# glmanhtu/vit-ed

Measured on NVIDIA B200. Metric: pair scores/sec (all-pairs ViT-ED), higher is better.
Workload: dtype fp16

## Files before the change

### vit-ed_b200/csrc/attention_tc.cu

```cuda
#include "kernels.h"

namespace vited {

namespace {

constexpr float kLog2e = 1.4426950408889634f;

__device__ __forceinline__ float ex2_ftz(float x) {
  float y;
  asm("ex2.approx.ftz.f32 %0, %1;" : "=f"(y) : "f"(x));
  return y;
}

struct P64 {
  static constexpr int HD = 32;
  static constexpr int RB = 64;
  static constexpr int TROWS = 80;
  static constexpr int TB = TROWS * RB;
  static constexpr int STAGE = 3 * TB;
  static constexpr int NS = 12;
  static constexpr int NT = 4;
  static constexpr int TCOLS = 128;
  static constexpr int OCOL = 96;
  static constexpr int THREADS = 32 * 4 * NT;
  static constexpr int BAR_BYTES = (2 * NS + 4 * NT) * 8 + 16;
  static constexpr int BYTES = 1024 + NS * STAGE + BAR_BYTES;
};

#ifdef VITED_ATTN_TRACE
__device__ unsigned long long g_p64_trace[4 * 64 * 8];
#define TRP(ev) do { if (blockIdx.x == 0 && quarter == 0 && lane == 0 && tk < 64) g_p64_trace[(group * 64 + tk) * 8 + (ev)] = clock64(); } while (0)
#else
#define TRP(ev) do { } while (0)
#endif

struct P64Maps {
  CUtensorMap q_tile, q_row, k_tile, k_row, v_tile, v_row;
};

__global__ void __launch_bounds__(P64::THREADS, 1)
attn_p64_kernel(AttnArgs a, const __grid_constant__ P64Maps maps, int n_units, int mode) {
  using C = P64;
  const int cls_only = mode & 1;
  const bool kv_once = (mode & 2) != 0;
  extern __shared__ uint8_t attn_tc_smem_raw[];
  uint8_t* smem = reinterpret_cast<uint8_t*>((reinterpret_cast<uintptr_t>(attn_tc_smem_raw) + 1023) & ~uintptr_t(1023));
  uint64_t* bars = reinterpret_cast<uint64_t*>(smem + C::NS * C::STAGE);
  uint64_t* full = bars;
  uint64_t* empty = bars + C::NS;
  uint64_t* s_full = bars + 2 * C::NS;
  uint64_t* o_full = s_full + C::NT;
  uint64_t* p_ready = o_full + C::NT;
  uint32_t* tmem_holder = reinterpret_cast<uint32_t*>(p_ready + C::NT);

  const int tid = threadIdx.x, lane = tid & 31;
  const int warp = __shfl_sync(0xffffffffu, tid >> 5, 0);
  const int quarter = warp & 3, group = warp >> 2;
  const int H = a.n_heads;
  const int n_my = (n_units - (int)blockIdx.x + (int)gridDim.x - 1) / (int)gridDim.x;
  const int NK = a.k_has_cls ? 80 : 64;

// ... 110 lines not shown
  } else {
    const float sl2 = a.scale * kLog2e;
    const int row = quarter * 32 + lane;
    const bool warp_active = quarter < 2 ? !cls_only : a.q_has_cls != 0;
    const uint32_t t_col = tmem_base + group * C::TCOLS;
    const uint32_t t_stage = t_col + (static_cast<uint32_t>(quarter * 32) << 16);
    uint32_t ph = 0;
    int tk = 0; (void)tk;
    for (int i = group; i < n_my; i += C::NT, ++tk) {
      const int u = (int)blockIdx.x + i * (int)gridDim.x;
      const int b = u / H, h = u - b * H;
      TRP(0);
      mbar_wait(&s_full[group], ph, 54);
      TRP(1);
      tc_fence_after();
      float l = 1.f;
      if (warp_active) {
        uint32_t v0[32], v1[32];
        uint32_t vc[8];
        tmem_ld_32x32b_x32(t_stage, v0);
        tmem_ld_32x32b_x32(t_stage + 32, v1);
        if (a.k_has_cls) tmem_ld_32x32b_x8(t_stage + 64, vc);
        tmem_ld_wait();
        float mx[4];
#pragma unroll
        for (int j = 0; j < 4; ++j) mx[j] = fmaxf(__uint_as_float(v0[j]), __uint_as_float(v1[j]));
#pragma unroll
        for (int j = 4; j < 32; ++j) mx[j & 3] = fmaxf(mx[j & 3], fmaxf(__uint_as_float(v0[j]), __uint_as_float(v1[j])));
        float mxa = fmaxf(fmaxf(mx[0], mx[1]), fmaxf(mx[2], mx[3]));
        if (a.k_has_cls) mxa = fmaxf(mxa, __uint_as_float(vc[0]));
        const float mneg = -mxa * sl2;
        float sum[4] = {0.f, 0.f, 0.f, 0.f};
        uint32_t pk[32];
#if VITED_SOFTMAX_PACKED
        {
          uint64_t sum2[2] = {0ull, 0ull};
          softmax_exp_pairs<16>(v0, sl2, mneg, pk, sum2);
          softmax_exp_pairs<16>(v1, sl2, mneg, pk + 16, sum2);
          f2_unpack(sum2[0], sum[0], sum[1]);
          f2_unpack(sum2[1], sum[2], sum[3]);
        }
#else
#pragma unroll
        for (int j = 0; j < 16; ++j) {
          const float p0 = ex2_ftz(fmaf(__uint_as_float(v0[2 * j]), sl2, mneg));
          const float p1 = ex2_ftz(fmaf(__uint_as_float(v0[2 * j + 1]), sl2, mneg));
          sum[(2 * j) & 3] += p0; sum[(2 * j + 1) & 3] += p1;
          pk[j] = pack_act(p0, p1);
        }
#pragma unroll
        for (int j = 0; j < 16; ++j) {
          const float p0 = ex2_ftz(fmaf(__uint_as_float(v1[2 * j]), sl2, mneg));
          const float p1 = ex2_ftz(fmaf(__uint_as_float(v1[2 * j + 1]), sl2, mneg));
          sum[(2 * j) & 3] += p0; sum[(2 * j + 1) & 3] += p1;
          pk[16 + j] = pack_act(p0, p1);
        }
#endif
        tmem_st_32x32b_x32(t_stage, pk);
        if (a.k_has_cls) {
          const float pc = ex2_ftz(fmaf(__uint_as_float(vc[0]), sl2, mneg));
          sum[0] += pc;
          uint32_t pc8[8] = {pack_act(pc, 0.f), 0u, 0u, 0u, 0u, 0u, 0u, 0u};
          tmem_st_32x32b_x8(t_stage + 32, pc8);
        }
        l = (sum[0] + sum[1]) + (sum[2] + sum[3]);
        tmem_st_wait();
      }
      tc_fence_before();
      __syncwarp();
      if (lane == 0) mbar_arrive(&p_ready[group]);
      TRP(2);
      mbar_wait(&o_full[group], ph, 55);
      TRP(3);
      tc_fence_after();
      if (warp_active) {
        uint32_t ov[32];
        tmem_ld_32x32b_x32(t_stage + C::OCOL, ov);
        tmem_ld_wait();
        const float inv = 1.f / l;
        size_t orow;
        bool valid = true;
        if (row < 64) { orow = (size_t)b * 64 + row; valid = !cls_only; }
        else if (row == 64 && a.q_has_cls) orow = (size_t)a.n_seq * 64 + b;
        else { valid = false; orow = 0; }
        if (valid) {
          uint4* dst = reinterpret_cast<uint4*>(a.o + orow * a.o_ld + h * C::HD);
#pragma unroll
          for (int c = 0; c < 4; ++c) {
            uint4 w;
            w.x = pack_act(__uint_as_float(ov[8 * c + 0]) * inv, __uint_as_float(ov[8 * c + 1]) * inv);
            w.y = pack_act(__uint_as_float(ov[8 * c + 2]) * inv, __uint_as_float(ov[8 * c + 3]) * inv);
            w.z = pack_act(__uint_as_float(ov[8 * c + 4]) * inv, __uint_as_float(ov[8 * c + 5]) * inv);
            w.w = pack_act(__uint_as_float(ov[8 * c + 6]) * inv, __uint_as_float(ov[8 * c + 7]) * inv);
            dst[c] = w;
          }
        }
      }
      TRP(4);
      ph ^= 1;
    }
  }

  tc_fence_before();
  __syncthreads();
  if (warp == 11) {
    tc_fence_after();
    tmem_dealloc(tmem_base, 512);
  }
}


struct L64 {
  static constexpr int HD = 64;
  static constexpr int RB = 128;
  static constexpr int QB = 128 * RB;
  static constexpr int KVB = 128 * RB;
  static constexpr int STAGE = 2 * KVB;
  static constexpr int NS = 4;
  static constexpr int THREADS = 352;
  static constexpr int GCOLS = 256;
  static constexpr int OCOL = 128;
  static constexpr int BAR_BYTES = 512;
  static constexpr int BYTES = 1024 + 4 * QB + NS * STAGE + BAR_BYTES;
};

#ifdef VITED_ATTN_TRACE
__device__ unsigned long long g_attn_trace[4 * 128 * 4];
#define TR(who, idx, k) do { if (blockIdx.x == 0 && lane == 0 && (idx) < 128) g_attn_trace[((who) * 128 + (idx)) * 4 + (k)] = clock64(); } while (0)
#else
#define TR(who, idx, k) do { } while (0)
#endif
// ... 337 lines not shown
  VITED_CHECK(items < ((size_t)1 << 31), "attention_tc: too many work items");
  static PerDeviceOnce once;
  const int sms = device_sm_count();
  if (once.first())
    VITED_CUDA_OK(cudaFuncSetAttribute(attn_l64_kernel, cudaFuncAttributeMaxDynamicSharedMemorySize, L64::BYTES));
  const uint64_t cols = (uint64_t)a.n_heads * 64;
  const uint64_t q_rows = (uint64_t)a.n_seq * a.nq_patch + (a.q_has_cls ? a.n_seq : 0);
  const uint64_t k_rows = (uint64_t)a.n_kv_seq * a.nk_patch + (a.k_has_cls ? a.n_kv_seq : 0);
  L64Maps maps;
  if (make_tmap_act_2d(&maps.q_tile, a.q, cols, q_rows, (uint64_t)a.q_ld * 2, 64, 128, 128)) return 1;
  if (make_tmap_act_2d(&maps.q_row, a.q, cols, q_rows, (uint64_t)a.q_ld * 2, 64, 1, 128)) return 1;
  if (make_tmap_act_2d(&maps.k_tile, a.k, cols, k_rows, (uint64_t)a.k_ld * 2, 64, 128, 128)) return 1;
  if (make_tmap_act_2d(&maps.k_row, a.k, cols, k_rows, (uint64_t)a.k_ld * 2, 64, 1, 128)) return 1;
  if (make_tmap_act_2d(&maps.v_tile, a.v, cols, k_rows, (uint64_t)a.v_ld * 2, 64, 128, 128)) return 1;
  if (make_tmap_act_2d(&maps.v_row, a.v, cols, k_rows, (uint64_t)a.v_ld * 2, 64, 1, 128)) return 1;
  const unsigned grid = (unsigned)(items < (size_t)sms ? items : (size_t)sms);
  VITED_CUDA_OK(launch_pdl(attn_l64_kernel, dim3(grid), dim3(L64::THREADS), L64::BYTES, stream, a, maps, (int)items));
  VITED_CUDA_OK(cudaGetLastError());
  return 0;
}

static int attention_tc_p64(const AttnArgs& a, int cls_only, cudaStream_t stream);

int attention_tc(const AttnArgs& a, cudaStream_t stream) {
  VITED_CHECK(attention_tc_supported(a), "attention_tc: unsupported shape");
  if (l64_shape(a)) return attention_tc_l64(a, stream);
#ifdef VITED_EXPERIMENTAL
  const char* pr = getenv("VITED_P64_PAIR");
  if (pr != nullptr && atoi(pr) != 0 && attention_pair_supported(a)) return attention_pair(a, stream);
#endif
  return attention_tc_p64(a, 0, stream);
}

bool attention_tc_cls_supported(const AttnArgs& a) { return a.n_heads >= 1 && p64_shape(a) && a.q_has_cls; }
int attention_tc_cls(const AttnArgs& a, cudaStream_t stream) {
  VITED_CHECK(attention_tc_cls_supported(a), "attention_tc_cls: unsupported shape");
  return attention_tc_p64(a, 1, stream);
}

static int attention_tc_p64(const AttnArgs& a, int cls_only, cudaStream_t stream) {
  const size_t units = (size_t)a.n_seq * a.n_heads;
  VITED_CHECK(units < ((size_t)1 << 31), "attention_tc: too many work units");
  static PerDeviceOnce once;
  const int sms = device_sm_count();
  if (once.first())
    VITED_CUDA_OK(cudaFuncSetAttribute(attn_p64_kernel, cudaFuncAttributeMaxDynamicSharedMemorySize, P64::BYTES));
  const uint64_t cols = (uint64_t)a.n_heads * 32;
  const uint64_t q_rows = (uint64_t)a.n_seq * 64 + (a.q_has_cls ? a.n_seq : 0);
  const uint64_t k_rows = (uint64_t)a.n_kv_seq * 64 + (a.k_has_cls ? a.n_kv_seq : 0);
  P64Maps maps;
  if (make_tmap_act_2d(&maps.q_tile, a.q, cols, q_rows, (uint64_t)a.q_ld * 2, 32, 64, 64)) return 1;
  if (make_tmap_act_2d(&maps.q_row, a.q, cols, q_rows, (uint64_t)a.q_ld * 2, 32, 1, 64)) return 1;
  if (make_tmap_act_2d(&maps.k_tile, a.k, cols, k_rows, (uint64_t)a.k_ld * 2, 32, 64, 64)) return 1;
// ... 23 lines not shown
```

### vit-ed_b200/csrc/engine.cu

```cuda
#include "../../include/vited_b200.h"
#include "kernels.h"

#include <cstdarg>
#include <cstdlib>
#include <cstring>
#include <map>
#include <string>
#include <vector>

namespace vited {

static thread_local char g_err[1024] = "";
void set_error(const char* fmt, ...) {
  va_list ap;
  va_start(ap, fmt);
  vsnprintf(g_err, sizeof(g_err), fmt, ap);
  va_end(ap);
}
const char* get_error() { return g_err; }

struct DevBuf {
  void* p = nullptr;
  size_t cap = 0;
  int ensure(size_t bytes) {
// ... 46 lines not shown
  std::vector<DecBlock> dec;
  LNorm norm;
  float* head_w = nullptr;
  float* head_b = nullptr;
  std::vector<void*> owned;
  std::map<std::string, Slot> slots;
  std::vector<std::string> names;
  int loaded = 0;
  int gemm_impl = IMPL_FAST, attn_impl = IMPL_FAST;
  int64_t chunk_rows = 524288;
  int cache_layer0 = 1;
  int prune_tail = 1;
  int fuse_ln = 1;
  int fuse_mlp = 1;
  int kv_budget_mb = 8000;
  int64_t launches = 0;
  int profile = 0;
  std::vector<cudaEvent_t> ev_pool;
  size_t ev_used = 0;
  struct ProfRec { cudaEvent_t ev; int cls; double flops; double bytes; };
  std::vector<ProfRec> recs;
  std::vector<std::string> cls_names;
  std::string profile_json;
  DevBuf x, h, qkv, o, q, delta, hid, col, tok, xsrc, enc_tok, kv, ci, xj, tmp_tok;

  int64_t workspace_bytes() const {
    return (int64_t)(x.cap + h.cap + qkv.cap + o.cap + q.cap + delta.cap + hid.cap + col.cap + tok.cap + xsrc.cap +
                     enc_tok.cap + kv.cap + ci.cap + xj.cap + tmp_tok.cap);
  }
};

namespace vited {

#define TRY(expr)            \
  do {                       \
    if ((expr) != 0) return 1; \
  } while (0)

static int alloc_f32(vited_engine* e, float** p, size_t n) {
  VITED_CUDA_OK(cudaMalloc(p, n * sizeof(float)));
  VITED_CUDA_OK(cudaMemset(*p, 0, n * sizeof(float)));
  e->owned.push_back(*p);
  return 0;
}
static int alloc_act(vited_engine* e, act_t** p, size_t n) {
  VITED_CUDA_OK(cudaMalloc(p, n * sizeof(act_t)));
  VITED_CUDA_OK(cudaMemset(*p, 0, n * sizeof(act_t)));
  e->owned.push_back(*p);
  return 0;
}
static void reg(vited_engine* e, const std::string& name, void* dst, bool to_act, int64_t numel) {
// ... 149 lines not shown
  a.x = x; a.delta = delta; a.gather_src = gsrc; a.gather_idx = gidx; a.gather_off = g_off; a.n_src_seq = n_src;
  a.ln_w = ln ? ln->w : nullptr; a.ln_b = ln ? ln->b : nullptr; a.h = h;
  a.n_seq = n_seq; a.n_patch = e->Ne; a.has_cls = has_cls; a.D = e->D; a.write_x = write_x; a.eps = 1e-6f;
  {
    const double rows = (double)n_seq * (e->Ne + (has_cls ? 1 : 0));
    const double per_row = e->D * (4.0 + (delta ? 2.0 : 0.0) + (write_x ? 4.0 : 0.0) + (ln ? 2.0 : 0.0));
    prof_mark(e, "resid_ln", 0.0, rows * per_row, s);
  }
  return resid_ln(a, s);
}
static int L_attn_self(vited_engine* e, const act_t* qkv, act_t* o, int n_seq, int has_cls, cudaStream_t s) {
  AttnArgs a;
  const int D = e->D;
  a.q = qkv; a.q_ld = 3 * D; a.k = qkv + D; a.k_ld = 3 * D; a.v = qkv + 2 * D; a.v_ld = 3 * D; a.o = o; a.o_ld = D;
  a.n_seq = n_seq; a.n_heads = e->H; a.head_dim = e->hd;
  a.nq_patch = e->Ne; a.q_has_cls = has_cls; a.nk_patch = e->Ne; a.k_has_cls = has_cls;
  a.n_kv_seq = n_seq; a.kv_index = nullptr; a.scale = e->scale;
  {
    const double n = e->Ne + (has_cls ? 1 : 0);
    prof_mark(e, "attn_self", 4.0 * n_seq * n * n * e->D, (double)n_seq * n * e->D * 2.0 * 4.0, s);
  }
  return attention(a, e->attn_impl, s);
}
static int L_attn_cross(vited_engine* e, const act_t* q, const act_t* kv, act_t* o, int n_seq, int n_kv_seq,
                        const int* kv_index, cudaStream_t s) {
  AttnArgs a;
  const int D = e->D;
  a.q = q; a.q_ld = D; a.k = kv; a.k_ld = 2 * D; a.v = kv + D; a.v_ld = 2 * D; a.o = o; a.o_ld = D;
  a.n_seq = n_seq; a.n_heads = e->H; a.head_dim = e->hd;
  a.nq_patch = e->Ne; a.q_has_cls = 1; a.nk_patch = e->Ne; a.k_has_cls = 0;
  a.n_kv_seq = n_kv_seq; a.kv_index = kv_index; a.scale = e->scale;
  prof_mark(e, "attn_cross", 4.0 * n_seq * (double)e->Nd * e->Ne * e->D, (double)n_seq * e->Nd * e->D * 2.0 * 2.0, s);
  return attention(a, e->attn_impl, s);
}

static int L_attn_cls(vited_engine* e, const act_t* q, int q_ld, const act_t* k, const act_t* v, int kv_ld, act_t* o,
                      int n_seq, int k_has_cls, int n_kv_seq, const int* kv_index, cudaStream_t s) {
  AttnArgs a;
  a.q = q; a.q_ld = q_ld; a.k = k; a.k_ld = kv_ld; a.v = v; a.v_ld = kv_ld; a.o = o; a.o_ld = e->D;
  a.n_seq = n_seq; a.n_heads = e->H; a.head_dim = e->hd;
  a.nq_patch = e->Ne; a.q_has_cls = 1; a.nk_patch = e->Ne; a.k_has_cls = k_has_cls;
  a.n_kv_seq = n_kv_seq; a.kv_index = kv_index; a.scale = e->scale;
  prof_mark(e, "attn_cls", 4.0 * n_seq * (double)(e->Ne + k_has_cls) * e->D,
            (double)n_seq * (e->Ne + k_has_cls) * e->D * 2.0 * 2.0, s);
  return attention_cls(a, s);
}
static int L_resid_ln_rows(vited_engine* e, float* x, const act_t* delta, const float* gsrc_cls_rows, const int* gidx,
                           const LNorm* ln, act_t* h, int rows, cudaStream_t s, int g_off = 0) {
  ResidLnArgs a;
  a.x = x; a.delta = delta; a.gather_src = gsrc_cls_rows; a.gather_idx = gidx; a.gather_off = g_off; a.n_src_seq = 0;
  a.ln_w = ln ? ln->w : nullptr; a.ln_b = ln ? ln->b : nullptr; a.h = h;
  a.n_seq = rows; a.n_patch = 1; a.has_cls = 0; a.D = e->D; a.write_x = 1; a.eps = 1e-6f;
  prof_mark(e, "resid_ln", 0.0, (double)rows * e->D * 12.0, s);
  return resid_ln(a, s);
// ... 115 lines not shown
                   s));
    TRY(L_gemm(e, e->h.as<act_t>(), b.kv, e->kv.as<act_t>() + l * per_layer, (int)rows, ACT_NONE, s));
  }
  return 0;
}

static int decode_chunk(vited_engine* e, int P, const int* ci, const int* xj, const float* xsrc, int n_src, int x_off,
                        int n_kv_seq, HeadArgs head, cudaStream_t s) {
  const size_t rows = (size_t)P * e->Nd;
  TRY(ensure_rows(e, rows));
  const size_t D = e->D;
  const size_t cls_off = (size_t)P * e->Ne;
  float* x = e->x.as<float>();
  act_t* h = e->h.as<act_t>();
  act_t* delta = e->delta.as<act_t>();
  act_t* qkv = e->qkv.as<act_t>();
  act_t* o = e->o.as<act_t>();
  act_t* q = e->q.as<act_t>();
  act_t* hid = e->hid.as<act_t>();
  const size_t kv_per_layer = (size_t)n_kv_seq * e->Ne * 2 * D;
  const size_t L = e->dec.size();
  const bool fuse = use_fused_ln(e, rows, e->dec[0].proj);
  bool h_is_norm1 = false;
  for (size_t l = 0; l < L; ++l) {
    DecBlock& b = e->dec[l];
    const bool first = (l == 0);
    const bool tail = e->prune_tail && (l + 1 == L);
    const act_t* kvl = e->kv.as<act_t>() + l * kv_per_layer;
    if (!tail) {
      if (first && e->cache_layer0) {
        TRY(L_resid_ln(e, x, nullptr, xsrc, xj, n_src, &b.norm_cross, h, P, 1, 1, s, x_off));
      } else {
        if (first) TRY(L_resid_ln(e, x, nullptr, xsrc, xj, n_src, &b.norm1, h, P, 1, 1, s, x_off));
        else if (!h_is_norm1) TRY(L_resid_ln(e, x, delta, nullptr, nullptr, 0, &b.norm1, h, P, 1, 1, s));
        TRY(L_gemm(e, h, b.qkv, qkv, (int)rows, ACT_NONE, s));
        TRY(L_attn_self(e, qkv, o, P, 1, s));
        if (fuse) {
          TRY(L_gemm_ln(e, o, b.proj, x, b.norm_cross, h, (int)rows, s));
        } else {
          TRY(L_gemm(e, o, b.proj, delta, (int)rows, ACT_NONE, s));
          TRY(L_resid_ln(e, x, delta, nullptr, nullptr, 0, &b.norm_cross, h, P, 1, 1, s));
        }
      }
      TRY(L_gemm(e, h, b.q, q, (int)rows, ACT_NONE, s));
      TRY(L_attn_cross(e, q, kvl, o, P, n_kv_seq, ci, s));
      h_is_norm1 = false;
      if (fuse && l + 1 < L && use_fused_mlp(e, rows, b.cproj, b.fc1, b.fc2)) {
        TRY(L_cproj_mlp_ln(e, o, b.cproj, b.norm2, b.fc1, b.fc2, x, e->dec[l + 1].norm1, h, (int)rows, s));
        h_is_norm1 = true;
      } else {
        if (fuse) {
          TRY(L_gemm_ln(e, o, b.cproj, x, b.norm2, h, (int)rows, s));
        } else {
          TRY(L_gemm(e, o, b.cproj, delta, (int)rows, ACT_NONE, s));
          TRY(L_resid_ln(e, x, delta, nullptr, nullptr, 0, &b.norm2, h, P, 1, 1, s));
        }
        if (fuse && l + 1 < L) {
          TRY(L_gemm(e, h, b.fc1, hid, (int)rows, ACT_GELU, s));
          TRY(L_gemm_ln(e, hid, b.fc2, x, e->dec[l + 1].norm1, h, (int)rows, s));
          h_is_norm1 = true;
        } else {
          TRY(L_gemm(e, h, b.fc1, hid, (int)rows, ACT_GELU, s));
          TRY(L_gemm(e, hid, b.fc2, delta, (int)rows, ACT_NONE, s));
        }
      }
    } else {
      float* x_c = x + cls_off * D;
      act_t* h_c = h + cls_off * D;
// ... 66 lines not shown
  VITED_CHECK(prop.major == 10, "vited_create: device %d is sm_%d%d; this library contains sm_100a code only", device,
              prop.major, prop.minor);
  vited_engine* e = new vited_engine();
  e->cfg = *cfg;
  e->device = device;
  const char* cr = getenv("VITED_CHUNK_ROWS");
  if (cr && atoll(cr) > 0) e->chunk_rows = atoll(cr);
  const char* fm = getenv("VITED_FUSE_MLP");
  if (fm) e->fuse_mlp = atoi(fm) ? 1 : 0;
  if (build(e) != 0) {
    vited_destroy(e);
    return 1;
  }
  *out = e;
  return 0;
}

void vited_destroy(vited_engine* e) {
  if (!e) return;
  DeviceScope scope(e->device);
  cudaDeviceSynchronize();
  for (void* p : e->owned) cudaFree(p);
  DevBuf* bufs[] = {&e->x, &e->h, &e->qkv, &e->o, &e->q, &e->delta, &e->hid, &e->col, &e->tok, &e->xsrc, &e->enc_tok,
                    &e->kv, &e->ci, &e->xj, &e->tmp_tok};
  for (DevBuf* b : bufs) b->release();
  for (cudaEvent_t ev : e->ev_pool) cudaEventDestroy(ev);
  delete e;
}

int vited_set_option(vited_engine* e, int option, int64_t value) {
  VITED_CHECK(e != nullptr, "null engine");
  switch (option) {
    case VITED_OPT_GEMM_IMPL: e->gemm_impl = value ? IMPL_REF : IMPL_FAST; return 0;
    case VITED_OPT_ATTN_IMPL: e->attn_impl = value == 1 ? IMPL_REF : value == 2 ? IMPL_MMA_SYNC : IMPL_FAST; return 0;
    case VITED_OPT_CHUNK_ROWS:
      VITED_CHECK(value >= 1, "chunk_rows must be positive");
      e->chunk_rows = value;
      return 0;
    case VITED_OPT_CACHE_LAYER0: e->cache_layer0 = value ? 1 : 0; return 0;
    case VITED_OPT_PRUNE_TAIL: e->prune_tail = value ? 1 : 0; return 0;
    case VITED_OPT_FUSE_LN: e->fuse_ln = value ? 1 : 0; return 0;
    case VITED_OPT_FUSE_MLP: e->fuse_mlp = value ? 1 : 0; return 0;
    case VITED_OPT_KV_BUDGET_MB:
      VITED_CHECK(value >= 1, "kv budget must be positive");
      e->kv_budget_mb = value;
      return 0;
    case VITED_OPT_PROFILE:
// ... 44 lines not shown
  for (int i0 = 0; i0 < B; i0 += step) {
    const int n = (B - i0 < step) ? (B - i0) : step;
    TRY(patch_tokens(e, images + (size_t)i0 * img, img, n, s));
    TRY(encoder_stack(e, n, out_tokens + (size_t)i0 * e->Ne * e->D, s));
  }
  return 0;
}

static int decode_impl(vited_engine* e, const float* ctx_tokens, const float* images, size_t img_stride, int B,
                       float* out_logits, cudaStream_t s) {
  const int step = items_per_batch(e);
  for (int i0 = 0; i0 < B; i0 += step) {
    const int n = (B - i0 < step) ? (B - i0) : step;
    TRY(patch_tokens(e, images + (size_t)i0 * img_stride, img_stride, n, s));
    TRY(decoder_item_state(e, n, s));
    TRY(e->xsrc.ensure((size_t)n * e->Nd * e->D * 4));
    VITED_CUDA_OK(cudaMemcpyAsync(e->xsrc.p, e->x.p, (size_t)n * e->Nd * e->D * 4, cudaMemcpyDeviceToDevice, s));
    TRY(build_kv(e, ctx_tokens + (size_t)i0 * e->Ne * e->D, n, s));
    size_t total = 0;
    TRY(build_pair_list(e, 2, 0, n, n, &total, s));
    HeadArgs head = {};
    head.out = out_logits + (size_t)i0 * e->C;
    head.ci = nullptr; head.xj = nullptr; head.row_begin = 0; head.n_items = 0;
    TRY(decode_chunk(e, n, e->ci.as<int>(), e->xj.as<int>(), e->xsrc.as<float>(), n, 0, n, head, s));
  }
  return 0;
}

int vited_decode(vited_engine* e, const float* ctx_tokens, const float* images, int B, float* out_logits,
                 void* stream) {
  TRY(check_ready(e));
  DeviceScope scope(e->device);
  VITED_CHECK(B >= 0 && (B == 0 || (ctx_tokens && images && out_logits)), "vited_decode: bad arguments");
  const size_t img = (size_t)e->cfg.in_chans * e->cfg.img_size * e->cfg.img_size;
  return decode_impl(e, ctx_tokens, images, img, B, out_logits, (cudaStream_t)stream);
}

int vited_forward_pairs(vited_engine* e, const float* pairs, int B, float* out_logits, void* stream) {
  TRY(check_ready(e));
  DeviceScope scope(e->device);
  VITED_CHECK(B >= 0 && (B == 0 || (pairs && out_logits)), "vited_forward_pairs: bad arguments");
  cudaStream_t s = (cudaStream_t)stream;
  const size_t img = (size_t)e->cfg.in_chans * e->cfg.img_size * e->cfg.img_size;
  const int step = items_per_batch(e);
  for (int i0 = 0; i0 < B; i0 += step) {
    const int n = (B - i0 < step) ? (B - i0) : step;
    const float* base = pairs + (size_t)i0 * 2 * img;
// ... 231 lines not shown
```

### vit-ed_b200/csrc/kernels.h

```cpp
#pragma once
#include "common.cuh"

namespace vited {

enum { ACT_NONE = 0, ACT_GELU = 1 };
enum { IMPL_FAST = 0, IMPL_REF = 1, IMPL_MMA_SYNC = 2 };

int gemm_act(const act_t* A, const act_t* W, const float* bias, act_t* C, int M, int N, int K, int act, int impl,
              cudaStream_t stream);
int gemm_num_sms();
int make_tmap_act_2d(CUtensorMap* tm, const void* ptr, uint64_t cols, uint64_t rows, uint64_t row_stride_bytes,
                      uint32_t box_cols, uint32_t box_rows, int swizzle_bytes);

int make_tmap_f32_2d(CUtensorMap* tm, const void* ptr, uint64_t cols, uint64_t rows, uint64_t row_stride_bytes,
                     uint32_t box_cols, uint32_t box_rows, int swizzle_bytes);

bool gemm_resid_ln_supported(int M, int N, int K);
int gemm_resid_ln(const act_t* A, const act_t* W, const float* bias, float* x, const float* ln_w, const float* ln_b,
                  act_t* h, int M, int N, int K, float eps, cudaStream_t stream);

bool mlp_resid_ln_supported(int M, int D, int hidden);
int mlp_resid_ln(const act_t* h_in, const act_t* W1, const float* b1, const act_t* W2, const float* b2, float* x,
                 const float* ln_w, const float* ln_b, act_t* h_out, int M, int D, int hidden, float eps,
                 cudaStream_t stream);
// ... 74 lines not shown
                           int src_row_off, int dst_block_stride, int dst_row_off, int D, float alpha, cudaStream_t s);
int train_attention(int backward, const act_t* q, int q_ld, const act_t* k, int k_ld, const act_t* v, int v_ld, act_t* o,
                    int o_ld, float* lse, const float* d_o, int do_ld, float* dsum, float* dq, int dq_ld, float* dk, int dk_ld,
                    float* dv, int dv_ld, int n_seq, int H, int hd, int Tq, int Tk, float scale, cudaStream_t s);
bool train_attention_wmma_supported(int hd);
int train_attention_wmma(int backward, const act_t* q, int q_ld, const act_t* k, int k_ld, const act_t* v, int v_ld, act_t* o,
                         int o_ld, float* lse, const float* d_o, int do_ld, float* dsum, float* dq, int dq_ld, float* dk,
                         int dk_ld, float* dv, int dv_ld, int n_seq, int H, int hd, int Tq, int Tk, float scale, cudaStream_t s);
int train_bce_logits(const float* logits, const float* labels, int n, float* loss, float* dlogits, float grad_scale,
                     cudaStream_t s);

struct AttnArgs {
  const act_t* q; int q_ld;
  const act_t* k; int k_ld;
  const act_t* v; int v_ld;
  act_t* o; int o_ld;
  int n_seq;
  int n_heads, head_dim;
  int nq_patch, q_has_cls;
  int nk_patch, k_has_cls;
  int n_kv_seq;
  const int* kv_index;
  float scale;
};
int attention(const AttnArgs& a, int impl, cudaStream_t stream);
bool attention_tc_supported(const AttnArgs& a);
int attention_tc(const AttnArgs& a, cudaStream_t stream);
bool attention_pair_supported(const AttnArgs& a);
int attention_pair(const AttnArgs& a, cudaStream_t stream);
bool attention_tc_cls_supported(const AttnArgs& a);
int attention_tc_cls(const AttnArgs& a, cudaStream_t stream);
int attention_cls(const AttnArgs& a, cudaStream_t stream);

}
```

Measured before the change: 345,100.

## Add context-unit cross-attention kernel batching queries that share a KV sequence

Result: no change. 344,600, median of 6 (-0.1%).

```diff
diff --git a/vit-ed_b200/csrc/attention_tc.cu b/vit-ed_b200/csrc/attention_tc.cu
--- a/vit-ed_b200/csrc/attention_tc.cu
+++ b/vit-ed_b200/csrc/attention_tc.cu
@@ -37,6 +37,96 @@
 struct P64Maps {
   CUtensorMap q_tile, q_row, k_tile, k_row, v_tile, v_row;
 };
+
+__device__ __forceinline__ float p64_row_max(const uint32_t (&v0)[32], const uint32_t (&v1)[32]) {
+  float mx[4];
+#pragma unroll
+  for (int j = 0; j < 4; ++j) mx[j] = fmaxf(__uint_as_float(v0[j]), __uint_as_float(v1[j]));
+#pragma unroll
+  for (int j = 4; j < 32; ++j) mx[j & 3] = fmaxf(mx[j & 3], fmaxf(__uint_as_float(v0[j]), __uint_as_float(v1[j])));
+  return fmaxf(fmaxf(mx[0], mx[1]), fmaxf(mx[2], mx[3]));
+}
+__device__ __forceinline__ void p64_row_exp(const uint32_t (&v0)[32], const uint32_t (&v1)[32], float sl2, float mneg,
+                                            uint32_t (&pk)[32], float (&sum)[4]) {
+#if VITED_SOFTMAX_PACKED
+  uint64_t sum2[2] = {0ull, 0ull};
+  softmax_exp_pairs<16>(v0, sl2, mneg, pk, sum2);
+  softmax_exp_pairs<16>(v1, sl2, mneg, pk + 16, sum2);
+  f2_unpack(sum2[0], sum[0], sum[1]);
+  f2_unpack(sum2[1], sum[2], sum[3]);
+#else
+#pragma unroll
+  for (int j = 0; j < 16; ++j) {
+    const float p0 = ex2_ftz(fmaf(__uint_as_float(v0[2 * j]), sl2, mneg));
+    const float p1 = ex2_ftz(fmaf(__uint_as_float(v0[2 * j + 1]), sl2, mneg));
+    sum[(2 * j) & 3] += p0; sum[(2 * j + 1) & 3] += p1;
+    pk[j] = pack_act(p0, p1);
+  }
+#pragma unroll
+  for (int j = 0; j < 16; ++j) {
+    const float p0 = ex2_ftz(fmaf(__uint_as_float(v1[2 * j]), sl2, mneg));
+    const float p1 = ex2_ftz(fmaf(__uint_as_float(v1[2 * j + 1]), sl2, mneg));
+    sum[(2 * j) & 3] += p0; sum[(2 * j + 1) & 3] += p1;
+    pk[16 + j] = pack_act(p0, p1);
+  }
+#endif
+}
+__device__ __forceinline__ float p64_row_max_tmem(uint32_t t_row) {
+  float mx[4];
+  uint32_t v[32];
+  tmem_ld_32x32b_x32(t_row, v);
+  tmem_ld_wait();
+#pragma unroll
+  for (int j = 0; j < 4; ++j) mx[j] = __uint_as_float(v[j]);
+#pragma unroll
+  for (int j = 4; j < 32; ++j) mx[j & 3] = fmaxf(mx[j & 3], __uint_as_float(v[j]));
+  tmem_ld_32x32b_x32(t_row + 32, v);
+  tmem_ld_wait();
+#pragma unroll
+  for (int j = 0; j < 32; ++j) mx[j & 3] = fmaxf(mx[j & 3], __uint_as_float(v[j]));
+  return fmaxf(fmaxf(mx[0], mx[1]), fmaxf(mx[2], mx[3]));
+}
+__device__ __forceinline__ void p64_row_exp_tmem(uint32_t t_row, float sl2, float mneg, float (&sum)[4]) {
+  asm volatile("" : "+r"(t_row) : "f"(mneg));
+#if VITED_SOFTMAX_PACKED
+  uint64_t sum2[2] = {0ull, 0ull};
+#endif
+#pragma unroll
+  for (int c = 0; c < 4; ++c) {
+    uint32_t v[16], pk[8];
+    tmem_ld_32x32b_x16(t_row + 16 * c, v);
+    tmem_ld_wait();
+#if VITED_SOFTMAX_PACKED
+    softmax_exp_pairs<8>(v, sl2, mneg, pk, sum2);
+#else
+#pragma unroll
+    for (int j = 0; j < 8; ++j) {
+      const float p0 = ex2_ftz(fmaf(__uint_as_float(v[2 * j]), sl2, mneg));
+      const float p1 = ex2_ftz(fmaf(__uint_as_float(v[2 * j + 1]), sl2, mneg));
+      sum[(2 * j) & 3] += p0; sum[(2 * j + 1) & 3] += p1;
+      pk[j] = pack_act(p0, p1);
+    }
+#endif
+    tmem_st_32x32b_x8(t_row + 8 * c, pk);
+  }
+#if VITED_SOFTMAX_PACKED
+  f2_unpack(sum2[0], sum[0], sum[1]);
+  f2_unpack(sum2[1], sum[2], sum[3]);
+#endif
+}
+__device__ __forceinline__ uint4 p64_pack8(const uint32_t* ov, float inv) {
+  uint4 w;
+  w.x = pack_act(__uint_as_float(ov[0]) * inv, __uint_as_float(ov[1]) * inv);
+  w.y = pack_act(__uint_as_float(ov[2]) * inv, __uint_as_float(ov[3]) * inv);
+  w.z = pack_act(__uint_as_float(ov[4]) * inv, __uint_as_float(ov[5]) * inv);
+  w.w = pack_act(__uint_as_float(ov[6]) * inv, __uint_as_float(ov[7]) * inv);
+  return w;
+}
+__device__ __forceinline__ void p64_store_row(act_t* o_row, const uint32_t (&ov)[32], float inv) {
+  uint4* dst = reinterpret_cast<uint4*>(o_row);
+#pragma unroll
+  for (int c = 0; c < 4; ++c) dst[c] = p64_pack8(ov + 8 * c, inv);
+}
 
 __global__ void __launch_bounds__(P64::THREADS, 1)
 attn_p64_kernel(AttnArgs a, const __grid_constant__ P64Maps maps, int n_units, int mode) {
@@ -193,40 +283,12 @@
         tmem_ld_32x32b_x32(t_stage + 32, v1);
         if (a.k_has_cls) tmem_ld_32x32b_x8(t_stage + 64, vc);
         tmem_ld_wait();
-        float mx[4];
-#pragma unroll
-        for (int j = 0; j < 4; ++j) mx[j] = fmaxf(__uint_as_float(v0[j]), __uint_as_float(v1[j]));
-#pragma unroll
-        for (int j = 4; j < 32; ++j) mx[j & 3] = fmaxf(mx[j & 3], fmaxf(__uint_as_float(v0[j]), __uint_as_float(v1[j])));
-        float mxa = fmaxf(fmaxf(mx[0], mx[1]), fmaxf(mx[2], mx[3]));
+        float mxa = p64_row_max(v0, v1);
         if (a.k_has_cls) mxa = fmaxf(mxa, __uint_as_float(vc[0]));
         const float mneg = -mxa * sl2;
         float sum[4] = {0.f, 0.f, 0.f, 0.f};
         uint32_t pk[32];
-#if VITED_SOFTMAX_PACKED
-        {
-          uint64_t sum2[2] = {0ull, 0ull};
-          softmax_exp_pairs<16>(v0, sl2, mneg, pk, sum2);
-          softmax_exp_pairs<16>(v1, sl2, mneg, pk + 16, sum2);
-          f2_unpack(sum2[0], sum[0], sum[1]);
-          f2_unpack(sum2[1], sum[2], sum[3]);
-        }
-#else
-#pragma unroll
-        for (int j = 0; j < 16; ++j) {
-          const float p0 = ex2_ftz(fmaf(__uint_as_float(v0[2 * j]), sl2, mneg));
-          const float p1 = ex2_ftz(fmaf(__uint_as_float(v0[2 * j + 1]), sl2, mneg));
-          sum[(2 * j) & 3] += p0; sum[(2 * j + 1) & 3] += p1;
-          pk[j] = pack_act(p0, p1);
-        }
-#pragma unroll
-        for (int j = 0; j < 16; ++j) {
-          const float p0 = ex2_ftz(fmaf(__uint_as_float(v1[2 * j]), sl2, mneg));
-          const float p1 = ex2_ftz(fmaf(__uint_as_float(v1[2 * j + 1]), sl2, mneg));
-          sum[(2 * j) & 3] += p0; sum[(2 * j + 1) & 3] += p1;
-          pk[16 + j] = pack_act(p0, p1);
-        }
-#endif
+        p64_row_exp(v0, v1, sl2, mneg, pk, sum);
         tmem_st_32x32b_x32(t_stage, pk);
         if (a.k_has_cls) {
           const float pc = ex2_ftz(fmaf(__uint_as_float(vc[0]), sl2, mneg));
@@ -254,18 +316,7 @@
         if (row < 64) { orow = (size_t)b * 64 + row; valid = !cls_only; }
         else if (row == 64 && a.q_has_cls) orow = (size_t)a.n_seq * 64 + b;
         else { valid = false; orow = 0; }
-        if (valid) {
-          uint4* dst = reinterpret_cast<uint4*>(a.o + orow * a.o_ld + h * C::HD);
-#pragma unroll
-          for (int c = 0; c < 4; ++c) {
-            uint4 w;
-            w.x = pack_act(__uint_as_float(ov[8 * c + 0]) * inv, __uint_as_float(ov[8 * c + 1]) * inv);
-            w.y = pack_act(__uint_as_float(ov[8 * c + 2]) * inv, __uint_as_float(ov[8 * c + 3]) * inv);
-            w.z = pack_act(__uint_as_float(ov[8 * c + 4]) * inv, __uint_as_float(ov[8 * c + 5]) * inv);
-            w.w = pack_act(__uint_as_float(ov[8 * c + 6]) * inv, __uint_as_float(ov[8 * c + 7]) * inv);
-            dst[c] = w;
-          }
-        }
+        if (valid) p64_store_row(a.o + orow * a.o_ld + h * C::HD, ov, inv);
       }
       TRP(4);
       ph ^= 1;
@@ -278,6 +329,278 @@
     tc_fence_after();
     tmem_dealloc(tmem_base, 512);
   }
+}
+
+struct P64Ctx {
+  static constexpr int HD = 32;
+  static constexpr int RB = 64;
+  static constexpr int QB = 128 * RB;
+  static constexpr int KB = 64 * RB;
+  static constexpr int STAGE = QB + 2 * KB;
+  static constexpr int NS = 12;
+  static constexpr int NT = 5;
+  static constexpr int TCOLS = 96;
+  static constexpr int OCOL = 64;
+  static constexpr int PRODUCER = 4 * NT, ISSUER = 4 * NT + 1;
+  static constexpr int THREADS = 32 * (4 * NT + 2);
+  static constexpr int BAR_BYTES = (2 * NS + 3 * NT) * 8 + 16;
+  static constexpr int BYTES = 1024 + NS * STAGE + BAR_BYTES;
+  static_assert(NT * TCOLS <= 512, "TMEM columns");
+};
+
+struct P64CtxMaps {
+  CUtensorMap q_tile, k_tile, v_tile;
+};
+
+__global__ void __launch_bounds__(P64Ctx::THREADS, 1)
+attn_p64_ctx_kernel(AttnArgs a, const __grid_constant__ P64CtxMaps maps) {
+  using C = P64Ctx;
+  constexpr int NT = C::NT;
+  extern __shared__ uint8_t attn_tc_smem_raw[];
+  uint8_t* smem = reinterpret_cast<uint8_t*>((reinterpret_cast<uintptr_t>(attn_tc_smem_raw) + 1023) & ~uintptr_t(1023));
+  uint64_t* bars = reinterpret_cast<uint64_t*>(smem + C::NS * C::STAGE);
+  uint64_t* full = bars;
+  uint64_t* empty = bars + C::NS;
+  uint64_t* s_full = bars + 2 * C::NS;
+  uint64_t* o_full = s_full + NT;
+  uint64_t* p_ready = o_full + NT;
+  uint32_t* tmem_holder = reinterpret_cast<uint32_t*>(p_ready + NT);
+
+  const int tid = threadIdx.x, lane = tid & 31;
+  const int warp = __shfl_sync(0xffffffffu, tid >> 5, 0);
+  const int quarter = warp & 3, group = warp >> 2;
+  const int H = a.n_heads;
+  const int4* units = reinterpret_cast<const int4*>(a.ctx_units) + 1;
+
+  if (tid == 0) {
+    for (int s = 0; s < C::NS; ++s) { mbar_init(&full[s], 1); mbar_init(&empty[s], 1); }
+    for (int t = 0; t < NT; ++t) {
+      mbar_init(&s_full[t], 1); mbar_init(&o_full[t], 1); mbar_init(&p_ready[t], 4);
+    }
+    fence_mbar_init();
+    tma_prefetch_desc(&maps.q_tile);
+    tma_prefetch_desc(&maps.k_tile);
+    tma_prefetch_desc(&maps.v_tile);
+  }
+  if (warp == C::ISSUER) {
+    tmem_alloc(tmem_holder, 512);
+    tmem_relinquish();
+  }
+  fence_proxy_async_smem();
+  tc_fence_before();
+  __syncthreads();
+  tc_fence_after();
+  const uint32_t tmem_base = *tmem_holder;
+  pdl_launch_dependents();
+  pdl_wait();
+
+  const int n_work = __ldg(a.ctx_units) * H;
+  const int n_my = (n_work - (int)blockIdx.x + (int)gridDim.x - 1) / (int)gridDim.x;
+
+  if (warp == C::PRODUCER) {
+    int s = 0;
+    uint32_t ph = 0;
+    for (int i0 = 0; i0 < n_my; i0 += 32) {
+      int4 my = make_int4(0, 0, 0, 0);
+      if (i0 + lane < n_my) my = __ldg(units + ((int)blockIdx.x + (i0 + lane) * (int)gridDim.x) / H);
+      const int jn = n_my - i0 < 32 ? n_my - i0 : 32;
+      for (int j = 0; j < jn; ++j) {
+        const int row0 = __shfl_sync(0xffffffffu, my.x, j);
+        const int rows = __shfl_sync(0xffffffffu, my.y, j);
+        const int kvb = __shfl_sync(0xffffffffu, my.z, j);
+        if (lane == 0) {
+          const int w = (int)blockIdx.x + (i0 + j) * (int)gridDim.x;
+          const int col = (w % H) * C::HD;
+          mbar_wait(&empty[s], ph ^ 1, 56);
+          uint8_t* st = smem + s * C::STAGE;
+          mbar_arrive_expect_tx(&full[s], (rows > 64 ? 2 : 1) * 64 * C::RB + 2 * C::KB);
+          tma_load_2d(&maps.q_tile, &full[s], st, col, row0);
+          if (rows > 64) tma_load_2d(&maps.q_tile, &full[s], st + 64 * C::RB, col, row0 + 64);
+          tma_load_2d(&maps.k_tile, &full[s], st + C::QB, col, kvb * 64);
+          tma_load_2d(&maps.v_tile, &full[s], st + C::QB + C::KB, col, kvb * 64);
+          if (++s == C::NS) { s = 0; ph ^= 1; }
+        }
+      }
+    }
+  } else if (warp == C::ISSUER) {
+    const uint32_t idesc_qk = umma_idesc_f16(128, 64);
+    const uint32_t idesc_pv = umma_idesc_f16(128, C::HD) | kIdescBMajorMN;
+    const uint32_t smem0 = smem_u32(smem);
+    auto issue_qk = [&](int i) {
+      const int s = i % C::NS, t = i % NT;
+      mbar_wait(&full[s], (uint32_t)(i / C::NS) & 1u, 57);
+      tc_fence_after();
+      const uint32_t q_addr = smem0 + s * C::STAGE;
+      const uint64_t dq = umma_desc_sw(q_addr, 64);
+      const uint64_t dk = umma_desc_sw(q_addr + C::QB, 64);
+      const uint32_t t_col = tmem_base + t * C::TCOLS;
+      if (elect_one_sync()) {
+#pragma unroll
+        for (int k = 0; k < C::HD / 16; ++k) umma_f16(t_col, dq + 2 * k, dk + 2 * k, idesc_qk, k);
+        umma_commit(&s_full[t]);
+      }
+      __syncwarp();
+    };
+    for (int i = 0; i < NT && i < n_my; ++i) issue_qk(i);
+    for (int i = 0; i < n_my; ++i) {
+      const int s = i % C::NS, t = i % NT;
+      const uint32_t t_col = tmem_base + t * C::TCOLS;
+      mbar_wait(&p_ready[t], (uint32_t)(i / NT) & 1u, 58);
+      tc_fence_after();
+      const uint64_t dv = umma_desc_sw(smem0 + s * C::STAGE + C::QB + C::KB, 64);
+      if (elect_one_sync()) {
+#pragma unroll
+        for (int k = 0; k < 4; ++k)
+          umma_f16_ts(t_col + C::OCOL, t_col + 8 * k, dv + 64 * k, idesc_pv, k);
+        umma_commit(&empty[s]);
+        umma_commit(&o_full[t]);
+      }
+      __syncwarp();
+      if (i + NT < n_my) issue_qk(i + NT);
+    }
+  } else {
+    const float sl2 = a.scale * kLog2e;
+    const int row = quarter * 32 + lane;
+    const uint32_t t_stage = tmem_base + group * C::TCOLS + (static_cast<uint32_t>(quarter * 32) << 16);
+    uint32_t ph = 0;
+    for (int w = (int)blockIdx.x + group * (int)gridDim.x; w < n_work; w += NT * (int)gridDim.x) {
+      const int h = w % H;
+      const int2 un = __ldg(reinterpret_cast<const int2*>(units + w / H));
+      const bool warp_active = quarter * 32 < un.y;
+      mbar_wait(&s_full[group], ph, 59);
+      tc_fence_after();
+      float l = 1.f;
+      if (warp_active) {
+        const float mneg = -p64_row_max_tmem(t_stage) * sl2;
+        float sum[4] = {0.f, 0.f, 0.f, 0.f};
+        p64_row_exp_tmem(t_stage, sl2, mneg, sum);
+        l = (sum[0] + sum[1]) + (sum[2] + sum[3]);
+        tmem_st_wait();
+      }
+      tc_fence_before();
+      __syncwarp();
+      if (lane == 0) mbar_arrive(&p_ready[group]);
+      mbar_wait(&o_full[group], ph, 60);
+      tc_fence_after();
+      if (warp_active) {
+        const float inv = 1.f / l;
+        uint4* dst = reinterpret_cast<uint4*>(a.o + (size_t)(un.x + row) * a.o_ld + h * C::HD);
+#pragma unroll
+        for (int c = 0; c < 2; ++c) {
+          uint32_t ov[16];
+          tmem_ld_32x32b_x16(t_stage + C::OCOL + 16 * c, ov);
+          tmem_ld_wait();
+          if (row < un.y) {
+            dst[2 * c] = p64_pack8(ov, inv);
+            dst[2 * c + 1] = p64_pack8(ov + 8, inv);
+          }
+        }
+      }
+      ph ^= 1;
+    }
+  }
+
+  tc_fence_before();
+  __syncthreads();
+  if (warp == C::ISSUER) {
+    tc_fence_after();
+    tmem_dealloc(tmem_base, 512);
+  }
+}
+
+constexpr int kUnitThreads = 1024, kUnitItems = 8, kUnitTile = kUnitThreads * kUnitItems;
+static_assert(kUnitTile % 128 == 0, "a tile boundary must be a class-token unit boundary");
+
+__device__ __forceinline__ int block_exclusive_scan(int v, int& total, int* sh) {
+  const int lane = threadIdx.x & 31, warp = threadIdx.x >> 5, nw = blockDim.x >> 5;
+  int x = v;
+#pragma unroll
+  for (int o = 1; o < 32; o <<= 1) {
+    const int y = __shfl_up_sync(0xffffffffu, x, o);
+    if (lane >= o) x += y;
+  }
+  if (lane == 31) sh[warp] = x;
+  __syncthreads();
+  if (warp == 0) {
+    int z = lane < nw ? sh[lane] : 0;
+#pragma unroll
+    for (int o = 1; o < 32; o <<= 1) {
+      const int y = __shfl_up_sync(0xffffffffu, z, o);
+      if (lane >= o) z += y;
+    }
+    sh[lane] = z;
+  }
+  __syncthreads();
+  const int r = (warp ? sh[warp - 1] : 0) + x - v;
+  total = sh[nw - 1];
+  __syncthreads();
+  return r;
+}
+
+__global__ void __launch_bounds__(kUnitThreads) ctx_units_kernel(const int* __restrict__ kv_index, int n_seq,
+                                                                 int q_has_cls, int4* __restrict__ out) {
+  __shared__ int sh[32];
+  __shared__ int starts[kUnitTile];
+  int base = 0;
+  const int T = (n_seq + 1) / 2;
+  for (int t0 = 0; t0 < T; t0 += kUnitTile) {
+    const int tb = t0 + (int)threadIdx.x * kUnitItems;
+    int k0[kUnitItems], k1[kUnitItems];
+    int cnt = 0;
+#pragma unroll
+    for (int j = 0; j < kUnitItems; ++j) {
+      const int t = tb + j;
+      k0[j] = t < T ? kv_index[2 * t] : 0;
+      k1[j] = 2 * t + 1 < n_seq ? kv_index[2 * t + 1] : k0[j];
+      cnt += t < T ? (k1[j] != k0[j] ? 2 : 1) : 0;
+    }
+    int total;
+    int pos = 1 + base + block_exclusive_scan(cnt, total, sh);
+#pragma unroll
+    for (int j = 0; j < kUnitItems; ++j) {
+      const int t = tb + j;
+      if (t >= T) break;
+      if (k1[j] == k0[j]) {
+        out[pos++] = make_int4(128 * t, 2 * t + 1 < n_seq ? 128 : 64, k0[j], 0);
+      } else {
+        out[pos++] = make_int4(128 * t, 64, k0[j], 0);
+        out[pos++] = make_int4(128 * t + 64, 64, k1[j], 0);
+      }
+    }
+    base += total;
+  }
+  for (int b0 = 0; q_has_cls && b0 < n_seq; b0 += kUnitTile) {
+    const int bb = b0 + (int)threadIdx.x * kUnitItems;
+    int k[kUnitItems];
+    int prev = bb % 128 != 0 && bb < n_seq ? kv_index[bb - 1] : 0;
+    uint32_t first = 0;
+#pragma unroll
+    for (int j = 0; j < kUnitItems; ++j) {
+      const int b = bb + j;
+      k[j] = b < n_seq ? kv_index[b] : 0;
+      if (b < n_seq && (b % 128 == 0 || k[j] != prev)) first |= 1u << j;
+      prev = k[j];
+    }
+    int total;
+    const int pos0 = block_exclusive_scan(__popc(first), total, sh);
+    int pos = pos0;
+#pragma unroll
+    for (int j = 0; j < kUnitItems; ++j)
+      if (first & (1u << j)) starts[pos++] = bb + j;
+    __syncthreads();
+    const int tile_end = n_seq - b0 < kUnitTile ? n_seq : b0 + kUnitTile;
+    pos = pos0;
+#pragma unroll
+    for (int j = 0; j < kUnitItems; ++j) {
+      if (first & (1u << j)) {
+        const int b = bb + j, e = pos + 1 < total ? starts[pos + 1] : tile_end;
+        out[1 + base + pos++] = make_int4(n_seq * 64 + b, e - b, k[j], 0);
+      }
+    }
+    base += total;
+    __syncthreads();
+  }
+  if (threadIdx.x == 0) out[0] = make_int4(base, 0, 0, 0);
 }
 
 
@@ -661,6 +984,66 @@
 
 static int attention_tc_p64(const AttnArgs& a, int cls_only, cudaStream_t stream);
 
+bool attention_ctx_enabled(const AttnArgs& a) {
+  if (!(a.n_heads >= 1 && p64_shape(a) && a.kv_index != nullptr && !a.k_has_cls)) return false;
+  const char* e = getenv("VITED_P64_CTX");
+  return e == nullptr || atoi(e) != 0;
+}
+
+size_t attention_ctx_units_bytes(int n_seq) { return (2 * (size_t)n_seq + 1) * sizeof(int4); }
+
+int attention_ctx_units(const int* kv_index, int n_seq, int q_has_cls, int* units, cudaStream_t stream) {
+  VITED_CHECK(n_seq >= 0 && (size_t)n_seq * 65 < ((size_t)1 << 31), "attention_ctx_units: bad n_seq %d", n_seq);
+  ctx_units_kernel<<<1, kUnitThreads, 0, stream>>>(kv_index, n_seq, q_has_cls, reinterpret_cast<int4*>(units));
+  VITED_CUDA_OK(cudaGetLastError());
+  return 0;
+}
+
+static int ctx_units_scratch(size_t bytes, int** p) {
+  static int* buf[64] = {};
+  static size_t cap[64] = {};
+  int d = 0;
+  VITED_CUDA_OK(cudaGetDevice(&d));
+  d &= 63;
+  if (cap[d] < bytes) {
+    if (buf[d]) VITED_CUDA_OK(cudaFree(buf[d]));
+    buf[d] = nullptr;
+    cap[d] = 0;
+    VITED_CUDA_OK(cudaMalloc(&buf[d], bytes));
+    cap[d] = bytes;
+  }
+  *p = buf[d];
+  return 0;
+}
+
+static int attention_tc_p64_ctx(const AttnArgs& a_in, cudaStream_t stream) {
+  using C = P64Ctx;
+  const size_t max_work = 2 * (size_t)a_in.n_seq * a_in.n_heads;
+  VITED_CHECK(max_work < ((size_t)1 << 31), "attention_tc: too many work units");
+  AttnArgs a = a_in;
+  if (a.ctx_units == nullptr) {
+    int* units = nullptr;
+    if (ctx_units_scratch(attention_ctx_units_bytes(a.n_seq), &units)) return 1;
+    if (attention_ctx_units(a.kv_index, a.n_seq, a.q_has_cls, units, stream)) return 1;
+    a.ctx_units = units;
+  }
+  static PerDeviceOnce once;
+  const int sms = device_sm_count();
+  if (once.first())
+    VITED_CUDA_OK(cudaFuncSetAttribute(attn_p64_ctx_kernel, cudaFuncAttributeMaxDynamicSharedMemorySize, C::BYTES));
+  const uint64_t cols = (uint64_t)a.n_heads * 32;
+  const uint64_t q_rows = (uint64_t)a.n_seq * 64 + (a.q_has_cls ? a.n_seq : 0);
+  const uint64_t k_rows = (uint64_t)a.n_kv_seq * 64;
+  P64CtxMaps maps;
+  if (make_tmap_act_2d(&maps.q_tile, a.q, cols, q_rows, (uint64_t)a.q_ld * 2, 32, 64, 64)) return 1;
+  if (make_tmap_act_2d(&maps.k_tile, a.k, cols, k_rows, (uint64_t)a.k_ld * 2, 32, 64, 64)) return 1;
+  if (make_tmap_act_2d(&maps.v_tile, a.v, cols, k_rows, (uint64_t)a.v_ld * 2, 32, 64, 64)) return 1;
+  const unsigned grid = (unsigned)(max_work < (size_t)sms ? max_work : (size_t)sms);
+  VITED_CUDA_OK(launch_pdl(attn_p64_ctx_kernel, dim3(grid), dim3(C::THREADS), C::BYTES, stream, a, maps));
+  VITED_CUDA_OK(cudaGetLastError());
+  return 0;
+}
+
 int attention_tc(const AttnArgs& a, cudaStream_t stream) {
   VITED_CHECK(attention_tc_supported(a), "attention_tc: unsupported shape");
   if (l64_shape(a)) return attention_tc_l64(a, stream);
@@ -668,6 +1051,7 @@
   const char* pr = getenv("VITED_P64_PAIR");
   if (pr != nullptr && atoi(pr) != 0 && attention_pair_supported(a)) return attention_pair(a, stream);
 #endif
+  if (attention_ctx_enabled(a)) return attention_tc_p64_ctx(a, stream);
   return attention_tc_p64(a, 0, stream);
 }
 
diff --git a/vit-ed_b200/csrc/engine.cu b/vit-ed_b200/csrc/engine.cu
--- a/vit-ed_b200/csrc/engine.cu
+++ b/vit-ed_b200/csrc/engine.cu
@@ -92,11 +92,11 @@
   std::vector<ProfRec> recs;
   std::vector<std::string> cls_names;
   std::string profile_json;
-  DevBuf x, h, qkv, o, q, delta, hid, col, tok, xsrc, enc_tok, kv, ci, xj, tmp_tok;
+  DevBuf x, h, qkv, o, q, delta, hid, col, tok, xsrc, enc_tok, kv, ci, xj, tmp_tok, ctx_units;
 
   int64_t workspace_bytes() const {
     return (int64_t)(x.cap + h.cap + qkv.cap + o.cap + q.cap + delta.cap + hid.cap + col.cap + tok.cap + xsrc.cap +
-                     enc_tok.cap + kv.cap + ci.cap + xj.cap + tmp_tok.cap);
+                     enc_tok.cap + kv.cap + ci.cap + xj.cap + tmp_tok.cap + ctx_units.cap);
   }
 };
 
@@ -292,14 +292,19 @@
   }
   return attention(a, e->attn_impl, s);
 }
-static int L_attn_cross(vited_engine* e, const act_t* q, const act_t* kv, act_t* o, int n_seq, int n_kv_seq,
-                        const int* kv_index, cudaStream_t s) {
+static AttnArgs cross_args(vited_engine* e, const act_t* q, const act_t* kv, act_t* o, int n_seq, int n_kv_seq,
+                           const int* kv_index, const int* ctx_units) {
   AttnArgs a;
   const int D = e->D;
   a.q = q; a.q_ld = D; a.k = kv; a.k_ld = 2 * D; a.v = kv + D; a.v_ld = 2 * D; a.o = o; a.o_ld = D;
   a.n_seq = n_seq; a.n_heads = e->H; a.head_dim = e->hd;
   a.nq_patch = e->Ne; a.q_has_cls = 1; a.nk_patch = e->Ne; a.k_has_cls = 0;
-  a.n_kv_seq = n_kv_seq; a.kv_index = kv_index; a.scale = e->scale;
+  a.n_kv_seq = n_kv_seq; a.kv_index = kv_index; a.scale = e->scale; a.ctx_units = ctx_units;
+  return a;
+}
+static int L_attn_cross(vited_engine* e, const act_t* q, const act_t* kv, act_t* o, int n_seq, int n_kv_seq,
+                        const int* kv_index, const int* ctx_units, cudaStream_t s) {
+  const AttnArgs a = cross_args(e, q, kv, o, n_seq, n_kv_seq, kv_index, ctx_units);
   prof_mark(e, "attn_cross", 4.0 * n_seq * (double)e->Nd * e->Ne * e->D, (double)n_seq * e->Nd * e->D * 2.0 * 2.0, s);
   return attention(a, e->attn_impl, s);
 }
@@ -461,6 +466,14 @@
   const size_t L = e->dec.size();
   const bool fuse = use_fused_ln(e, rows, e->dec[0].proj);
   bool h_is_norm1 = false;
+  const int* ctx_units = nullptr;
+  if (e->attn_impl == IMPL_FAST && (L > 1 || !e->prune_tail) &&
+      attention_ctx_enabled(cross_args(e, q, e->kv.as<act_t>(), o, P, n_kv_seq, ci, nullptr))) {
+    TRY(e->ctx_units.ensure(attention_ctx_units_bytes(P)));
+    prof_mark(e, "attn_units", 0.0, (double)P * 4.0 * 2.0 + attention_ctx_units_bytes(P), s);
+    TRY(attention_ctx_units(ci, P, 1, e->ctx_units.as<int>(), s));
+    ctx_units = e->ctx_units.as<int>();
+  }
   for (size_t l = 0; l < L; ++l) {
     DecBlock& b = e->dec[l];
     const bool first = (l == 0);
@@ -482,7 +495,7 @@
         }
       }
       TRY(L_gemm(e, h, b.q, q, (int)rows, ACT_NONE, s));
-      TRY(L_attn_cross(e, q, kvl, o, P, n_kv_seq, ci, s));
+      TRY(L_attn_cross(e, q, kvl, o, P, n_kv_seq, ci, ctx_units, s));
       h_is_norm1 = false;
       if (fuse && l + 1 < L && use_fused_mlp(e, rows, b.cproj, b.fc1, b.fc2)) {
         TRY(L_cproj_mlp_ln(e, o, b.cproj, b.norm2, b.fc1, b.fc2, x, e->dec[l + 1].norm1, h, (int)rows, s));
@@ -595,7 +608,7 @@
   cudaDeviceSynchronize();
   for (void* p : e->owned) cudaFree(p);
   DevBuf* bufs[] = {&e->x, &e->h, &e->qkv, &e->o, &e->q, &e->delta, &e->hid, &e->col, &e->tok, &e->xsrc, &e->enc_tok,
-                    &e->kv, &e->ci, &e->xj, &e->tmp_tok};
+                    &e->kv, &e->ci, &e->xj, &e->tmp_tok, &e->ctx_units};
   for (DevBuf* b : bufs) b->release();
   for (cudaEvent_t ev : e->ev_pool) cudaEventDestroy(ev);
   delete e;
@@ -686,7 +699,7 @@
     HeadArgs head = {};
     head.out = out_logits + (size_t)i0 * e->C;
     head.ci = nullptr; head.xj = nullptr; head.row_begin = 0; head.n_items = 0;
-    TRY(decode_chunk(e, n, e->ci.as<int>(), e->xj.as<int>(), e->xsrc.as<float>(), n, 0, n, head, s));
+    TRY(decode_chunk(e, n, nullptr, e->xj.as<int>(), e->xsrc.as<float>(), n, 0, n, head, s));
   }
   return 0;
 }
diff --git a/vit-ed_b200/csrc/kernels.h b/vit-ed_b200/csrc/kernels.h
--- a/vit-ed_b200/csrc/kernels.h
+++ b/vit-ed_b200/csrc/kernels.h
@@ -120,12 +120,16 @@
   int n_kv_seq;
   const int* kv_index;
   float scale;
+  const int* ctx_units = nullptr;
 };
 int attention(const AttnArgs& a, int impl, cudaStream_t stream);
 bool attention_tc_supported(const AttnArgs& a);
 int attention_tc(const AttnArgs& a, cudaStream_t stream);
 bool attention_pair_supported(const AttnArgs& a);
 int attention_pair(const AttnArgs& a, cudaStream_t stream);
+bool attention_ctx_enabled(const AttnArgs& a);
+size_t attention_ctx_units_bytes(int n_seq);
+int attention_ctx_units(const int* kv_index, int n_seq, int q_has_cls, int* units, cudaStream_t stream);
 bool attention_tc_cls_supported(const AttnArgs& a);
 int attention_tc_cls(const AttnArgs& a, cudaStream_t stream);
 int attention_cls(const AttnArgs& a, cudaStream_t stream);
```
